# tkonolige/city2ba

Hardware: AMD Instinct MI355X
Metric: million observations/sec (project+Jacobian) (higher is better)
Workload: dtype f64

## Files before the change

city2ba_amd/csrc/capi_problem.hpp:

```cpp


struct c2b_problem {
    int device = 0;
    hipStream_t stream = nullptr;
    int64_t n_cam = 0, n_pts = 0, n_obs = 0;
    DevBuf<double> cam15, bal9, camblk, cen4, pts4, uv;
    DevBuf<uint32_t> cam_idx, pt_idx;
    DevBuf<char> ws;
    DevBuf<double> stats, scalar;
    int64_t shard_cam_base = 0, shard_n_cam_global = -1, shard_obs_base = 0;
    c2b_problem_options opt{0, 0, 0, 0, 0, 0, -1};
    int loss_kind = 0;
    double loss_scale = 1.0;
    int precond_kind = 0;
    int64_t precond_fallbacks = 0;
    DevBuf<uint16_t> cmask;
    DevBuf<uint8_t> pmask;
    std::vector<uint16_t> h_cmask;
    std::vector<uint8_t> h_pmask;
    int64_t const_n_cam = -1, const_n_pts = -1, const_params = 0, const_pts = 0;
    bool bal_valid = false;
    bool blk_valid = false;
    bool bal9_fresh = false;
    DevBuf<uint64_t> rows_ptr;
// ... 1273 lines not shown
    if (cam_lo < 0 || cam_hi < cam_lo || cam_hi > p->n_cam)
        return fail(C2B_ERR_INVALID_ARGUMENT, "problem_export_device: camera range [%lld, %lld) outside [0, %lld]", (long long)cam_lo,
                    (long long)cam_hi, (long long)p->n_cam);
    int rc = ensure_rows(p);
    if (rc) return rc;
    hipStream_t st = p->stream;
    uint64_t ends[2] = {0, 0};
    if (p->n_obs) {
        HIP_TRY(hipMemcpyAsync(&ends[0], p->rows_ptr + cam_lo, sizeof(uint64_t), hipMemcpyDeviceToHost, st));
        HIP_TRY(hipMemcpyAsync(&ends[1], p->rows_ptr + cam_hi, sizeof(uint64_t), hipMemcpyDeviceToHost, st));
        HIP_TRY(hipStreamSynchronize(st));
    }
    const int64_t o0 = (int64_t)ends[0], n = (int64_t)(ends[1] - ends[0]), nc = cam_hi - cam_lo;
    if (obs_lo) *obs_lo = o0;
    if (n_obs_slice) *n_obs_slice = n;
    if (cam15 && nc) HIP_TRY(hipMemcpyAsync(cam15, p->cam15 + 15 * cam_lo, sizeof(double) * 15 * (size_t)nc, hipMemcpyDeviceToDevice, st));
    if (pts4 && p->n_pts) HIP_TRY(hipMemcpyAsync(pts4, p->pts4, sizeof(double) * 4 * (size_t)p->n_pts, hipMemcpyDeviceToDevice, st));
    if (row_ptr) {
        if (p->n_obs) {
            hipLaunchKernelGGL(k_rows_rebase, dim3(blocks_of(nc + 1, 256)), dim3(256), 0, st, (const uint64_t *)(p->rows_ptr + cam_lo), nc + 1,
                               ends[0], row_ptr);
            LAUNCH_CHECK();
        } else {
            HIP_TRY(hipMemsetAsync(row_ptr, 0, sizeof(uint64_t) * (size_t)(nc + 1), st));
        }
    }
    if (pt_idx && n) HIP_TRY(hipMemcpyAsync(pt_idx, p->pt_idx + o0, sizeof(uint32_t) * (size_t)n, hipMemcpyDeviceToDevice, st));
    if (uv && n) HIP_TRY(hipMemcpyAsync(uv, p->uv + 2 * o0, sizeof(double) * 2 * (size_t)n, hipMemcpyDeviceToDevice, st));
    HIP_TRY(hipStreamSynchronize(st));
    return C2B_OK;
    C2B_API_END("problem_export_device")
}

static hipError_t compact_rows_on_device(c2b_problem *p, const uint64_t *d_row_old, const uint8_t *d_keep, const uint32_t *d_pt,
                                         const double *d_uv, int64_t n_cam, uint64_t *row_ptr_host, DevBuf<uint64_t> &row_new,
                                         DevBuf<uint32_t> &pt_new, DevBuf<double> &uv_new, int64_t *w) {
    DevBuf<uint64_t> d_tot;
    *w = 0;
    hipError_t e = d_tot.alloc((size_t)n_cam + 1);
    if (e == hipSuccess) e = row_new.alloc((size_t)n_cam + 1);
    if (e != hipSuccess) return e;
    const unsigned row_blocks = (unsigned)((n_cam + 3) / 4);
    if (n_cam) hipLaunchKernelGGL(k_keep_row_counts, dim3(row_blocks), dim3(256), 0, p->stream, d_row_old, d_keep, n_cam, d_tot);
    hipLaunchKernelGGL(k_dense_cam_scan, dim3(1), dim3(256), 0, p->stream, (const uint64_t *)d_tot, n_cam, row_new);
    e = hipMemcpyAsync(row_ptr_host, row_new, sizeof(uint64_t) * (size_t)(n_cam + 1), hipMemcpyDeviceToHost, p->stream);
    if (e == hipSuccess) e = hipStreamSynchronize(p->stream);
    if (e != hipSuccess) return e;
    *w = (int64_t)row_ptr_host[n_cam];
    e = pt_new.alloc((size_t)*w);
    if (e == hipSuccess) e = uv_new.alloc(2 * (size_t)*w);
    if (e == hipSuccess && n_cam) {
        hipLaunchKernelGGL(k_keep_row_scatter, dim3(row_blocks), dim3(256), 0, p->stream, d_row_old, (const uint64_t *)row_new, d_keep,
                           d_pt, reinterpret_cast<const double2 *>(d_uv), n_cam, pt_new, reinterpret_cast<double2 *>(uv_new.ptr));
        e = launch_error();
    }
    if (e == hipSuccess) e = hipStreamSynchronize(p->stream);
    return e;
}

int c2b_problem_visibility_pairs_compact(c2b_problem *p, int64_t n_pairs, const uint32_t *cam_idx, const uint32_t *pt_idx,
                                         double max_dist, uint64_t *row_ptr) {
    C2B_API_BEGIN
    NEED_UPLOADED(p, "problem_visibility_pairs_compact");
    if (n_pairs < 0 || !row_ptr || (n_pairs && (!cam_idx || !pt_idx)))
        return fail(C2B_ERR_INVALID_ARGUMENT, "problem_visibility_pairs_compact: bad arguments");
    for (int64_t i = 0; i < n_pairs; ++i) {
        if (cam_idx[i] >= (uint64_t)p->n_cam || pt_idx[i] >= (uint64_t)p->n_pts)
            return fail(C2B_ERR_INDEX_OUT_OF_RANGE, "problem_visibility_pairs_compact: pair %lld out of range", (long long)i);
        if (i && cam_idx[i] < cam_idx[i - 1])
            return fail(C2B_ERR_INVALID_ARGUMENT, "problem_visibility_pairs_compact: cam_idx must be non-decreasing (pair %lld)", (long long)i);
    }
    int rc = ensure_camblk(p);
    if (rc) return rc;
    free_dense(p);
    const int64_t n_cam = p->n_cam;
    const size_t n = (size_t)(n_pairs ? n_pairs : 1);
    DevBuf<uint32_t> d_c, d_p, d_pt_new;
    DevBuf<double> d_uv, d_uv_new;
    DevBuf<uint8_t> d_k;
    DevBuf<uint64_t> d_row, d_row_new;
    int64_t w = 0;
    hipError_t e = d_c.alloc(n);
    if (e == hipSuccess) e = d_p.alloc(n);
    if (e == hipSuccess) e = d_uv.alloc(2 * n);
    if (e == hipSuccess) e = d_k.alloc(n);
    if (e == hipSuccess) e = d_row.alloc((size_t)n_cam + 1);
    if (e == hipSuccess && n_pairs) e = hipMemcpyAsync(d_c, cam_idx, sizeof(uint32_t) * n, hipMemcpyHostToDevice, p->stream);
    if (e == hipSuccess && n_pairs) e = hipMemcpyAsync(d_p, pt_idx, sizeof(uint32_t) * n, hipMemcpyHostToDevice, p->stream);
    if (e == hipSuccess) {
        if (n_pairs) rc = c2b_visibility_pairs(p->camblk, p->pts4, d_c, d_p, n_pairs, max_dist, d_uv, d_k, p->stream);
        if (!rc) {
            hipLaunchKernelGGL(k_rows_from_sorted, dim3(blocks_for(n_pairs + 1)), dim3(kBlock), 0, p->stream, (const uint32_t *)d_c,
                               n_pairs, n_cam, d_row);
            e = launch_error();
            if (e == hipSuccess)
                e = compact_rows_on_device(p, d_row, d_k, d_p, d_uv, n_cam, row_ptr, d_row_new, d_pt_new, d_uv_new, &w);
        }
    }
    if (rc || e != hipSuccess) (void)hipStreamSynchronize(p->stream);
    if (!rc && e == hipSuccess) {
        p->dense_row = std::move(d_row_new); p->dense_pt = std::move(d_pt_new); p->dense_uv = std::move(d_uv_new); p->dense_n = w;
    }
    if (rc) return rc;
    if (e != hipSuccess) return fail(hip_code(e), "problem_visibility_pairs_compact: %s", hipGetErrorString(e));
    return C2B_OK;
    C2B_API_END("problem_visibility_pairs_compact")
}

int c2b_problem_visibility_within_distance(c2b_problem *p, double max_dist, int occlusion, double block_length, double block_inset,
                                           uint64_t *row_ptr) {
    C2B_API_BEGIN
    NEED_UPLOADED(p, "problem_visibility_within_distance");
    if (!(max_dist >= 0.0) || (occlusion && !(block_length > 0.0)))
        return fail(C2B_ERR_INVALID_ARGUMENT, "problem_visibility_within_distance: max_dist must be >= 0 (and block_length > 0 with occlusion)");
    const int64_t n_cam = p->n_cam, n_pts = p->n_pts;
    if (n_pts >= ((int64_t)1 << 32) || n_cam >= ((int64_t)1 << 31))
        return fail(C2B_ERR_INVALID_ARGUMENT, "problem_visibility_within_distance: too many cameras or points");
    int rc = ensure_camblk(p);
    if (rc) return rc;
    free_dense(p);
    hipStream_t st = p->stream;
    if (n_cam == 0 || n_pts == 0) {
        DevBuf<uint64_t> row0;
        DevBuf<uint32_t> pt0;
        DevBuf<double> uv0;
        hipError_t e0 = row0.alloc((size_t)n_cam + 1);
        if (e0 == hipSuccess) e0 = pt0.alloc(1);
        if (e0 == hipSuccess) e0 = uv0.alloc(2);
        if (e0 == hipSuccess) e0 = hipMemsetAsync(row0.ptr, 0, sizeof(uint64_t) * (size_t)(n_cam + 1), st);
        if (e0 == hipSuccess) e0 = hipStreamSynchronize(st);
        if (e0 != hipSuccess) return fail(C2B_ERR_HIP, "problem_visibility_within_distance: %s", hipGetErrorString(e0));
        if (row_ptr) std::fill(row_ptr, row_ptr + n_cam + 1, (uint64_t)0);
        p->dense_row = std::move(row0); p->dense_pt = std::move(pt0); p->dense_uv = std::move(uv0);
        p->dense_n = 0;
        return C2B_OK;
    }
    double stats[C2B_STATS_DOUBLES];
    rc = compute_stats(p);
    if (rc) return rc;
    HIP_TRY(hipMemcpyAsync(stats, p->stats, sizeof stats, hipMemcpyDeviceToHost, st));
    HIP_TRY(hipStreamSynchronize(st));
    CellGrid g;
    g.x0 = stats[6]; g.z0 = stats[8];
    const double ex = stats[9] - stats[6], ez = stats[11] - stats[8];
    double cs = (max_dist > 0.0 ? max_dist : 1.0) * (1.0 + 0x1.0p-20);
    if (!(ex >= 0.0) || !(ez >= 0.0) || !std::isfinite(ex) || !std::isfinite(ez) || !std::isfinite(cs))
        return fail(C2B_ERR_INVALID_ARGUMENT, "problem_visibility_within_distance: non-finite coordinates");
    auto cells = [&](double c) { return (std::floor(ex / c) + 1.0) * (std::floor(ez / c) + 1.0); };
    while (cells(cs) > (double)(1 << 24)) cs *= 2.0;
    g.inv_cs = 1.0 / cs;
    g.ncx = (int)std::floor(ex / cs) + 1; g.ncz = (int)std::floor(ez / cs) + 1;
    const int64_t n_cells = (int64_t)g.ncx * g.ncz;

    DevArena arena;
    DevBuf<uint32_t> cell_of, counts, cursor, sorted, tiles, total, cam_count, pos, max32;
    DevBuf<unsigned long long> sum64;
    DevBuf<uint64_t> row64;
    const int64_t big = std::max(n_cells + 1, n_cam + 1);
    auto temporaries = [&](auto &&each) {
        each(cell_of, (size_t)n_pts); each(counts, (size_t)(n_cells + 1)); each(cursor, (size_t)(n_cells + 1));
        each(sorted, (size_t)n_pts); each(tiles, (size_t)(big / kScanTile + 2)); each(total, (size_t)1);
        each(cam_count, (size_t)(n_cam + 1)); each(pos, (size_t)(n_cam + 1)); each(sum64, (size_t)1); each(max32, (size_t)1);
    };
    size_t arena_bytes = 0;
    temporaries([&](auto &b, size_t n) { arena_bytes += DevArena::room(b, n); });
    hipError_t e = arena.reserve(arena_bytes);
    if (e == hipSuccess) e = row64.alloc((size_t)n_cam + 1);
    if (e != hipSuccess) return fail(hip_code(e), "problem_visibility_within_distance: %s", hipGetErrorString(e));
    temporaries([&](auto &b, size_t n) { arena.carve(b, n); });

    HIP_TRY(hipMemsetAsync(counts.ptr, 0, 4 * (size_t)(n_cells + 1), st));
    HIP_TRY(hipMemsetAsync(cursor.ptr, 0, 4 * (size_t)(n_cells + 1), st));
    HIP_TRY(hipMemsetAsync(cam_count.ptr, 0, 4 * (size_t)(n_cam + 1), st));
    HIP_TRY(hipMemsetAsync(sum64.ptr, 0, 8, st));
    HIP_TRY(hipMemsetAsync(max32.ptr, 0, 4, st));
    if (n_pts) hipLaunchKernelGGL(k_cells_assign, dim3(blocks_of(n_pts, 256)), dim3(256), 0, st, reinterpret_cast<const double4 *>(p->pts4.ptr), n_pts,
                                  g, cell_of, counts);
    uint32_t n_sorted = 0, n_kept32 = 0;
    uint32_t *start = cursor;
    e = scan_flags(st, counts, n_cells + 1, start, tiles, total, &n_sorted);
    if (e == hipSuccess && (int64_t)n_sorted != n_pts) return fail(C2B_ERR_HIP, "problem_visibility_within_distance: cell counts do not add up");
    if (e == hipSuccess) e = hipMemsetAsync(counts.ptr, 0, 4 * (size_t)(n_cells + 1), st);
    if (e == hipSuccess && n_pts)
        hipLaunchKernelGGL(k_cells_fill, dim3(blocks_of(n_pts, 256)), dim3(256), 0, st, cell_of, n_pts,
                           (const uint32_t *)start, counts, sorted);
    const unsigned cam_blocks = blocks_of(n_cam, kCellWPB);
    if (e == hipSuccess && n_cam && n_pts) {
        hipLaunchKernelGGL((k_cells_visibility<false>), dim3(cam_blocks), dim3(kCellWPB * 64), 0, st, (const double *)p->camblk, n_cam,
                           reinterpret_cast<const double4 *>(p->pts4.ptr), g, (const uint32_t *)start, sorted,
                           max_dist, occlusion ? 1 : 0, block_length, block_inset, cam_count, (const uint64_t *)nullptr,
                           (uint32_t *)nullptr, (double2 *)nullptr);
        hipLaunchKernelGGL(k_sum_u32_u64, dim3(256), dim3(256), 0, st, cam_count, n_cam, sum64);
        hipLaunchKernelGGL(k_max_u32, dim3(256), dim3(256), 0, st, cam_count, n_cam, max32);
    }
    if (e == hipSuccess) e = scan_flags(st, cam_count, n_cam + 1, pos, tiles, total, &n_kept32);
    unsigned long long n_kept = 0;
    uint32_t longest = 0;
    if (e == hipSuccess) e = hipMemcpy(&n_kept, sum64.ptr, 8, hipMemcpyDeviceToHost);
    if (e == hipSuccess) e = hipMemcpy(&longest, max32.ptr, 4, hipMemcpyDeviceToHost);
    if (e == hipSuccess && n_kept != (unsigned long long)n_kept32)
        return fail(C2B_ERR_INVALID_ARGUMENT, "problem_visibility_within_distance: more than 2^32 observations");
    if (e == hipSuccess) {
        hipLaunchKernelGGL(k_widen_u32, dim3(blocks_for(n_cam + 1)), dim3(kBlock), 0, st, pos, n_cam + 1, row64);
        e = launch_error();
    }
    DevBuf<uint32_t> tmp_pt, out_pt;
    DevBuf<double2> tmp_uv;
    DevBuf<double> out_uv;
    const size_t w = (size_t)n_kept;
    if (e == hipSuccess) e = tmp_pt.alloc(w);
    if (e == hipSuccess) e = tmp_uv.alloc(w);
    if (e == hipSuccess) e = out_pt.alloc(w);
    if (e == hipSuccess) e = out_uv.alloc(2 * w);
    if (e == hipSuccess && w) {
        hipLaunchKernelGGL((k_cells_visibility<true>), dim3(cam_blocks), dim3(kCellWPB * 64), 0, st, (const double *)p->camblk, n_cam,
                           reinterpret_cast<const double4 *>(p->pts4.ptr), g, (const uint32_t *)start, sorted,
                           max_dist, occlusion ? 1 : 0, block_length, block_inset, (uint32_t *)nullptr, row64,
                           tmp_pt, tmp_uv);
        const uint32_t long_row = p->opt.rank_sort_max_row > 0 ? (uint32_t)p->opt.rank_sort_max_row : 2048u;
        if (longest <= long_row) {
            hipLaunchKernelGGL(k_rows_rank_sort, dim3(cam_blocks), dim3(kCellWPB * 64), 0, st, row64, n_cam, tmp_pt, tmp_uv, out_pt,
                               reinterpret_cast<double2 *>(out_uv.ptr));
            e = launch_error();
        } else {
            e = launch_error();
            std::vector<uint64_t> rp((size_t)n_cam + 1);
            std::vector<uint32_t> hp(w), hq(w);
            std::vector<double> hu(2 * w), hv(2 * w);
            if (e == hipSuccess) e = hipMemcpyAsync(rp.data(), row64.ptr, 8 * ((size_t)n_cam + 1), hipMemcpyDeviceToHost, st);
            if (e == hipSuccess) e = hipMemcpyAsync(hp.data(), tmp_pt.ptr, 4 * w, hipMemcpyDeviceToHost, st);
            if (e == hipSuccess) e = hipMemcpyAsync(hu.data(), tmp_uv.ptr, 16 * w, hipMemcpyDeviceToHost, st);
            if (e == hipSuccess) e = hipStreamSynchronize(st);
            if (e == hipSuccess) {
                const int T = (int)std::min<int64_t>(std::max(1u, std::thread::hardware_concurrency()), std::max<int64_t>(1, n_cam));
                c2b_host::run_threads(T, [&](int t) {
                        std::vector<uint32_t> order;
                        for (int64_t c = n_cam * t / T; c < n_cam * (t + 1) / T; ++c) {
                            const size_t b = (size_t)rp[(size_t)c], k = (size_t)(rp[(size_t)c + 1] - rp[(size_t)c]);
                            order.resize(k);
                            for (size_t i = 0; i < k; ++i) order[i] = (uint32_t)i;
                            std::sort(order.begin(), order.end(), [&](uint32_t x, uint32_t y) { return hp[b + x] < hp[b + y]; });
                            for (size_t i = 0; i < k; ++i) {
                                hq[b + i] = hp[b + order[i]];
                                hv[2 * (b + i)] = hu[2 * (b + order[i])];
                                hv[2 * (b + i) + 1] = hu[2 * (b + order[i]) + 1];
                            }
                        }
                    });
                e = hipMemcpyAsync(out_pt.ptr, hq.data(), 4 * w, hipMemcpyHostToDevice, st);
                if (e == hipSuccess) e = hipMemcpyAsync(out_uv.ptr, hv.data(), 16 * w, hipMemcpyHostToDevice, st);
                if (e == hipSuccess) e = hipStreamSynchronize(st);
            }
        }
    }
    if (e == hipSuccess && row_ptr)
        e = hipMemcpyAsync(row_ptr, row64.ptr, sizeof(uint64_t) * (size_t)(n_cam + 1), hipMemcpyDeviceToHost, st);
    if (e == hipSuccess) e = hipStreamSynchronize(st);
    if (e != hipSuccess) {
        (void)hipStreamSynchronize(st);
        return fail(hip_code(e), "problem_visibility_within_distance: %s", hipGetErrorString(e));
    }
    p->dense_row = std::move(row64); p->dense_pt = std::move(out_pt); p->dense_uv = std::move(out_uv);
    p->dense_n = (int64_t)n_kept;
    return C2B_OK;
    C2B_API_END("problem_visibility_within_distance")
}

int c2b_problem_generate_world_points(c2b_problem *p, const float *tri9, int64_t n_tri, int64_t num_points, double max_dist,
                                      uint64_t seed, int64_t *n_out) {
    C2B_API_BEGIN
    NEED_UPLOADED(p, "problem_generate_world_points");
    if (!tri9 || n_tri < 0 || num_points < 0 || !n_out || num_points >= ((int64_t)1 << 31))
        return fail(C2B_ERR_INVALID_ARGUMENT, "problem_generate_world_points: bad arguments");
    if (p->n_obs != 0) return fail(C2B_ERR_INVALID_ARGUMENT, "problem_generate_world_points: the problem already has observations");
    if (p->n_cam == 0)
        return fail(C2B_ERR_INVALID_ARGUMENT, "Cannot generate world points with 0 cameras. Try increasing the number of cameras generated (via --cameras).");
    if (n_tri == 0) return fail(C2B_ERR_INVALID_ARGUMENT, "the model has no triangles");
    int rc = ensure_camblk(p);
    if (rc) return rc;
    hipStream_t st = p->stream;
    const int64_t n_cam = p->n_cam;
    std::vector<double> cum((size_t)n_tri);
    {
        double acc = 0.0;
        for (int64_t t = 0; t < n_tri; ++t) {
            const float *q = tri9 + 9 * t;
            const double a[3] = {(double)q[3] - (double)q[0], (double)q[4] - (double)q[1], (double)q[5] - (double)q[2]};
            const double b[3] = {(double)q[6] - (double)q[0], (double)q[7] - (double)q[1], (double)q[8] - (double)q[2]};
            const double c[3] = {a[1] * b[2] - a[2] * b[1], a[2] * b[0] - a[0] * b[2], a[0] * b[1] - a[1] * b[0]};
            acc += std::sqrt((c[0] * c[0] + c[1] * c[1]) + c[2] * c[2]) / 2.0;
            cum[(size_t)t] = acc;
        }
    }
    DevBuf<float> d_tri;
    DevBuf<double> d_cum;
    const double4 *centres = reinterpret_cast<const double4 *>(p->cen4.ptr);
    hipError_t e = d_tri.alloc(9 * (size_t)n_tri);
    if (e == hipSuccess) e = d_cum.alloc((size_t)n_tri);
    if (e == hipSuccess) e = hipMemcpyAsync(d_tri.ptr, tri9, 36 * (size_t)n_tri, hipMemcpyHostToDevice, st);
    if (e == hipSuccess) e = hipMemcpyAsync(d_cum.ptr, cum.data(), 8 * (size_t)n_tri, hipMemcpyHostToDevice, st);
    if (e != hipSuccess) return fail(hip_code(e), "problem_generate_world_points: %s", hipGetErrorString(e));
    double stats[C2B_STATS_DOUBLES];
    rc = c2b_stats(p->camblk, p->cen4, n_cam, p->pts4, 0, p->ws, p->stats, st);
    if (rc) return rc;
    HIP_TRY(hipMemcpyAsync(stats, p->stats, sizeof stats, hipMemcpyDeviceToHost, st));
    HIP_TRY(hipStreamSynchronize(st));
    CellGrid g;
    g.x0 = stats[6]; g.z0 = stats[8];
    const double ex = stats[9] - stats[6], ez = stats[11] - stats[8];
    double cs = (max_dist > 0.0 ? max_dist : 1.0) * (1.0 + 0x1.0p-20);
    if (!(ex >= 0.0) || !(ez >= 0.0) || !std::isfinite(ex) || !std::isfinite(ez) || !std::isfinite(cs))
        return fail(C2B_ERR_INVALID_ARGUMENT, "problem_generate_world_points: non-finite coordinates");
    auto cells = [&](double c) { return (std::floor(ex / c) + 1.0) * (std::floor(ez / c) + 1.0); };
    while (cells(cs) > (double)(1 << 24)) cs *= 2.0;
    g.inv_cs = 1.0 / cs;
    g.ncx = (int)std::floor(ex / cs) + 1; g.ncz = (int)std::floor(ez / cs) + 1;
    const int64_t n_cells = (int64_t)g.ncx * g.ncz;
    const int64_t chunk = std::max<int64_t>(4096, std::min<int64_t>(num_points, (int64_t)1 << 20));
    DevBuf<uint32_t> cell_of, counts, startb, sorted, tiles, total, ok, pos;
    DevBuf<double4> cand;
    DevBuf<unsigned long long> cutoff;
    DevBuf<double> out;
    const int64_t big = std::max(n_cells + 1, chunk);
    e = cell_of.alloc((size_t)n_cam);
    if (e == hipSuccess) e = counts.alloc((size_t)(n_cells + 1));
    if (e == hipSuccess) e = startb.alloc((size_t)(n_cells + 1));
    if (e == hipSuccess) e = sorted.alloc((size_t)n_cam);
    if (e == hipSuccess) e = tiles.alloc((size_t)(big / kScanTile + 2));
    if (e == hipSuccess) e = total.alloc(1);
    if (e == hipSuccess) e = cand.alloc((size_t)chunk);
    if (e == hipSuccess) e = ok.alloc((size_t)chunk);
    if (e == hipSuccess) e = pos.alloc((size_t)chunk);
    if (e == hipSuccess) e = cutoff.alloc(1);
    if (e == hipSuccess) e = out.alloc(4 * (size_t)std::max<int64_t>(num_points, 1));
    if (e == hipSuccess) e = hipMemsetAsync(counts.ptr, 0, 4 * (size_t)(n_cells + 1), st);
    if (e != hipSuccess) return fail(hip_code(e), "problem_generate_world_points: %s", hipGetErrorString(e));
    hipLaunchKernelGGL(k_cells_assign, dim3(blocks_of(n_cam, 256)), dim3(256), 0, st, centres, n_cam, g, cell_of, counts);
    uint32_t n_sorted = 0;
    e = scan_flags(st, counts, n_cells + 1, startb, tiles, total, &n_sorted);
    if (e == hipSuccess && (int64_t)n_sorted != n_cam) return fail(C2B_ERR_HIP, "problem_generate_world_points: cell counts do not add up");
    if (e == hipSuccess) e = hipMemsetAsync(counts.ptr, 0, 4 * (size_t)(n_cells + 1), st);
    if (e == hipSuccess)
        hipLaunchKernelGGL(k_cells_fill, dim3(blocks_of(n_cam, 256)), dim3(256), 0, st, cell_of, n_cam, startb, counts, sorted);
    if (e == hipSuccess) e = launch_error();
    int64_t accepted = 0, failed = 0;
    const int64_t fail_threshold = 10 * num_points;
    for (int64_t k0 = 0; e == hipSuccess && accepted < num_points && failed < fail_threshold; k0 += chunk) {
        const unsigned long long all = (unsigned long long)chunk;
        e = hipMemcpyAsync(cutoff.ptr, &all, 8, hipMemcpyHostToDevice, st);
        if (e != hipSuccess) break;
        hipLaunchKernelGGL(k_world_candidates, dim3(blocks_of(chunk, 256)), dim3(256), 0, st, d_tri, n_tri, d_cum, seed, k0, chunk,
                           centres, g, startb, sorted, max_dist, cand, ok);
        uint32_t n_ok = 0;
        e = scan_flags(st, ok, chunk, pos, tiles, total, &n_ok);
        if (e != hipSuccess) break;
        hipLaunchKernelGGL(k_world_cutoff, dim3(blocks_of(chunk, 256)), dim3(256), 0, st, pos, chunk,
                           (uint64_t)(num_points - accepted), (uint64_t)(fail_threshold - failed), cutoff);
        hipLaunchKernelGGL(k_world_accept, dim3(blocks_of(chunk, 256)), dim3(256), 0, st, cand, ok, pos, chunk, cutoff,
                           reinterpret_cast<double4 *>(out.ptr) + accepted);
        e = launch_error();
        unsigned long long cut = 0;
        if (e == hipSuccess) e = hipMemcpyAsync(&cut, cutoff.ptr, 8, hipMemcpyDeviceToHost, st);
        if (e == hipSuccess) e = hipStreamSynchronize(st);
        if (e != hipSuccess) break;
        uint32_t took = n_ok;
        if ((int64_t)cut < chunk) {
            e = hipMemcpy(&took, pos + cut, 4, hipMemcpyDeviceToHost);
            if (e != hipSuccess) break;
        }
        accepted += (int64_t)took;
        failed += (int64_t)cut - (int64_t)took;
    }
    if (e != hipSuccess) return fail(C2B_ERR_HIP, "problem_generate_world_points: %s", hipGetErrorString(e));
    if (failed >= fail_threshold && num_points > 0)
        return fail(C2B_ERR_INVALID_ARGUMENT, "Failed to generate enough points. %lld successes, %lld failures, %lld requested points.",
// ... 348 lines not shown
```

city2ba_amd/csrc/cell_kernels.hpp:

```cpp
#pragma once
#include "camera_math.hpp"

namespace c2b {

struct CellGrid {
    double x0, z0, inv_cs;
    int ncx, ncz;
};

C2B_DEV int cell_coord(double v, double v0, double inv_cs, int n) {
    const double f = floor((v - v0) * inv_cs);
    return f < 0.0 ? 0 : (f >= (double)n ? n - 1 : (int)f);
}

__global__ __launch_bounds__(256) void k_cells_assign(const double4 *__restrict__ pts4, int64_t n, CellGrid g,
                                                     uint32_t *__restrict__ cell_of, uint32_t *__restrict__ counts) {
    const int64_t j = (int64_t)blockIdx.x * 256 + threadIdx.x;
    if (j >= n) return;
    const double4 p = pts4[j];
    const uint32_t c = (uint32_t)(cell_coord(p.x, g.x0, g.inv_cs, g.ncx) * g.ncz + cell_coord(p.z, g.z0, g.inv_cs, g.ncz));
    cell_of[j] = c;
    atomicAdd(counts + c, 1u);
}

__global__ __launch_bounds__(256) void k_cells_fill(const uint32_t *__restrict__ cell_of, int64_t n, const uint32_t *__restrict__ start,
                                                   uint32_t *__restrict__ cursor, uint32_t *__restrict__ sorted) {
    const int64_t j = (int64_t)blockIdx.x * 256 + threadIdx.x;
    if (j >= n) return;
    const uint32_t c = cell_of[j];
    sorted[start[c] + atomicAdd(cursor + c, 1u)] = (uint32_t)j;
}

C2B_DEV bool seg_unique_intersection(double p0x, double p0y, double p1x, double p1y, double q0x, double q0y, double q1x,
                                     double q1y, double &ix, double &iy) {
    const double rx = p1x - p0x, ry = p1y - p0y;
    const double sx = q1x - q0x, sy = q1y - q0y;
    const double r_cross_s = rx * sy - ry * sx;
    if (r_cross_s == 0.0) return false;
    const double qpx = q0x - p0x, qpy = q0y - p0y;
    const double t = qpx * (sy / r_cross_s) - qpy * (sx / r_cross_s);
    const double u = qpx * (ry / r_cross_s) - qpy * (rx / r_cross_s);
    if (!(0.0 <= t && t <= 1.0 && 0.0 <= u && u <= 1.0)) return false;
    ix = p0x + t * rx;
    iy = p0y + t * ry;
    return true;
}

C2B_DEV bool hits_in_block_dev(double sx, double sy, double ex, double ey, int64_t bix, int64_t biy, double L, double inset) {
    const double block_end = L - inset;
    const double ox = (double)bix * L, oy = (double)biy * L;
    const double lo_x = ox + inset, lo_y = oy + inset, hi_x = ox + block_end, hi_y = oy + block_end;
#pragma unroll
    for (int k = 0; k < 4; ++k) {
        const double ax = k == 2 ? hi_x : lo_x, ay = k == 3 ? hi_y : lo_y;
        const double bx = k == 0 ? lo_x : hi_x, by = k == 1 ? lo_y : hi_y;
        double px, py;
        if (seg_unique_intersection(sx, sy, ex, ey, ax, ay, bx, by, px, py)) {
            const double dx = ex - px;
            if (sqrt(dx * dx + (ey - py)) > 1e-8) return true;
        }
    }
    return false;
}

C2B_DEV bool hits_building_dev(double cx, double cz, double px, double pz, double L, double inset) {
    const int64_t cbx = (int64_t)trunc(cx / L), cby = (int64_t)trunc(cz / L);
    const int64_t pbx = (int64_t)trunc(px / L), pby = (int64_t)trunc(pz / L);
    const int64_t x0 = cbx < pbx ? cbx : pbx, x1 = cbx < pbx ? pbx : cbx;
    const int64_t y0 = cby < pby ? cby : pby, y1 = cby < pby ? pby : cby;
    for (int64_t bx = x0; bx <= x1; ++bx)
        for (int64_t by = y0; by <= y1; ++by)
            if (hits_in_block_dev(cx, cz, px, pz, bx, by, L, inset)) return true;
    return false;
}

constexpr int kCellWPB = 4;
template <bool FILL>
__global__ __launch_bounds__(kCellWPB * 64) void k_cells_visibility(
    const double *__restrict__ camblk, int64_t n_cam, const double4 *__restrict__ pts4, CellGrid g,
    const uint32_t *__restrict__ start, const uint32_t *__restrict__ sorted, double max_dist, int occlusion, double L,
    double inset, uint32_t *__restrict__ cam_count, const uint64_t *__restrict__ row_ptr, uint32_t *__restrict__ pt_out,
    double2 *__restrict__ uv_out) {
    const int lane = threadIdx.x & 63;
    const int64_t c = (int64_t)blockIdx.x * kCellWPB + __builtin_amdgcn_readfirstlane(threadIdx.x >> 6);
    if (c >= n_cam) return;
    const CamRec cam(camblk, c);
    const double gx = cam[kCenter], gy = cam[kCenter + 1], gz = cam[kCenter + 2];
    const int ccx = cell_coord(gx, g.x0, g.inv_cs, g.ncx), ccz = cell_coord(gz, g.z0, g.inv_cs, g.ncz);
    const double r2 = max_dist * max_dist;
    uint64_t dst = FILL ? row_ptr[c] : 0;
    uint32_t count = 0;
    const int ix0 = ccx > 0 ? ccx - 1 : 0, ix1 = ccx + 1 < g.ncx ? ccx + 1 : g.ncx - 1;
    const int iz0 = ccz > 0 ? ccz - 1 : 0, iz1 = ccz + 1 < g.ncz ? ccz + 1 : g.ncz - 1;
    for (int ix = ix0; ix <= ix1; ++ix) {
        const uint32_t b = start[ix * g.ncz + iz0], e = start[ix * g.ncz + iz1 + 1];
        for (uint32_t k0 = b; k0 < e; k0 += 64) {
            const uint32_t k = k0 + lane;
            const bool valid = k < e;
            const uint32_t j = sorted[valid ? k : e - 1];
            const double4 X = pts4[j];
            const double dx = gx - X.x, dy = gy - X.y, dz = gz - X.z;
            const double d2 = dot3(dx, dy, dz, dx, dy, dz);
            bool keep = valid && d2 <= r2;
            double u = 0.0, v = 0.0;
            if (keep) {
                const Proj p = project_obs(cam, X.x, X.y, X.z);
                u = p.u; v = p.v;
                keep = sqrt(d2) < max_dist && p.qz <= 0.0 && u >= -1.0 && u <= 1.0 && v >= -1.0 && v <= 1.0;
            }
            if (keep && occlusion) keep = !hits_building_dev(gx, gz, X.x, X.z, L, inset);
            const uint64_t m = __builtin_amdgcn_ballot_w64(keep);
            if (FILL && keep) {
                const uint64_t at = dst + (uint64_t)__builtin_popcountll(m & ((1ull << lane) - 1ull));
                pt_out[at] = j;
                uv_out[at] = make_double2(u, v);
            }
            const uint32_t got = (uint32_t)__builtin_popcountll(m);
            count += got;
            dst += got;
        }
    }
    if (!FILL && lane == 0) cam_count[c] = count;
}

__global__ __launch_bounds__(kCellWPB * 64) void k_rows_rank_sort(const uint64_t *__restrict__ row_ptr, int64_t n_cam,
                                                                const uint32_t *__restrict__ pt_in, const double2 *__restrict__ uv_in,
                                                                uint32_t *__restrict__ pt_out, double2 *__restrict__ uv_out) {
    const int lane = threadIdx.x & 63;
    const int64_t c = (int64_t)blockIdx.x * kCellWPB + __builtin_amdgcn_readfirstlane(threadIdx.x >> 6);
    if (c >= n_cam) return;
    const uint64_t b = row_ptr[c], e = row_ptr[c + 1];
    for (uint64_t i0 = b; i0 < e; i0 += 64) {
        const uint64_t i = i0 + lane;
        const bool valid = i < e;
        const uint32_t mine = pt_in[valid ? i : e - 1];
        uint32_t rank = 0;
        for (uint64_t j = b; j < e; ++j) rank += pt_in[j] < mine ? 1u : 0u;
        if (valid) {
            pt_out[b + rank] = mine;
            uv_out[b + rank] = uv_in[i];
        }
    }
}

__global__ __launch_bounds__(256) void k_max_u32(const uint32_t *__restrict__ v, int64_t n, uint32_t *__restrict__ out) {
    uint32_t m = 0;
    for (int64_t i = (int64_t)blockIdx.x * 256 + threadIdx.x; i < n; i += (int64_t)gridDim.x * 256) m = v[i] > m ? v[i] : m;
#pragma unroll
    for (int off = 32; off > 0; off >>= 1) { const uint32_t o = __shfl_down(m, off, 64); m = o > m ? o : m; }
    if ((threadIdx.x & 63) == 0 && m) atomicMax(out, m);
}

__global__ __launch_bounds__(256) void k_sum_u32_u64(const uint32_t *__restrict__ v, int64_t n, unsigned long long *__restrict__ out) {
    unsigned long long s = 0;
    for (int64_t i = (int64_t)blockIdx.x * 256 + threadIdx.x; i < n; i += (int64_t)gridDim.x * 256) s += v[i];
#pragma unroll
    for (int off = 32; off > 0; off >>= 1) s += __shfl_down(s, off, 64);
    if ((threadIdx.x & 63) == 0 && s) atomicAdd(out, s);
}

struct GridDirs { double m[4][9]; };

C2B_DEV void grid_slot(int64_t n, int64_t B, int64_t slots, int per, int64_t &bx, int64_t &by, int64_t &i, int &k, bool &along_x) {
    const int64_t row_full = slots * per * (2 * B + 1);
    if (n < B * row_full) {
        bx = n / row_full;
        const int64_t r = n % row_full;
        if (r < 2 * per * slots * B) {
            by = r / (2 * per * slots);
            const int64_t r2 = r % (2 * per * slots);
            i = r2 / (2 * per);
            const int kk = (int)(r2 % (2 * per));
            along_x = kk < per; k = kk % per;
        } else {
            by = B;
            const int64_t r2 = r - 2 * per * slots * B;
            i = r2 / per; k = (int)(r2 % per); along_x = true;
        }
    } else {
        bx = B;
        const int64_t r = n - B * row_full;
        by = r / (per * slots);
        const int64_t r2 = r % (per * slots);
        i = r2 / per; k = (int)(r2 % per); along_x = false;
    }
}

__global__ __launch_bounds__(256) void k_grid_cameras(int64_t n_cam, int64_t cpb, int64_t B, double L, double cam_h, GridDirs d,
                                                     double *__restrict__ cam15) {
    const int64_t n = (int64_t)blockIdx.x * 256 + threadIdx.x;
    if (n >= n_cam) return;
    int64_t bx, by, i;
    int k;
    bool along_x;
    grid_slot(n, B, cpb, 2, bx, by, i, k, along_x);
    const double offset_x = L * (double)bx, offset_z = L * (double)by;
    const double t = (double)i / (double)cpb * L;
    const double px = along_x ? offset_x + t : offset_x, pz = along_x ? offset_z : offset_z + t;
    const double *R = d.m[(along_x ? 0 : 2) + k];
    double v[3];
    cm_mat_vec(R, px, cam_h, pz, v);
    double *o = cam15 + 15 * n;
#pragma unroll
    for (int q = 0; q < 9; ++q) o[q] = R[q];
    o[9] = -1.0 * v[0]; o[10] = -1.0 * v[1]; o[11] = -1.0 * v[2];
    o[12] = 1.0; o[13] = 0.0; o[14] = 0.0;
}

__global__ __launch_bounds__(256) void k_grid_points(int64_t n_pts, int64_t ppb, int64_t B, double L, double inset, double pt_h,
                                                    double4 *__restrict__ pts4) {
    const int64_t n = (int64_t)blockIdx.x * 256 + threadIdx.x;
    if (n >= n_pts) return;
    int64_t bx, by, i;
    int k;
    bool along_x;
    grid_slot(n, B, ppb, 6, bx, by, i, k, along_x);
    const double offset_x = L * (double)bx, offset_z = L * (double)by;
    const double step = (L - inset * 2.0) / (double)ppb;
    const double loc = (along_x ? offset_x : offset_z) + inset + (double)i * step;
    const double a = k < 2 ? loc : loc + step / 2.0;
    const double o = along_x ? offset_z : offset_x;
    const double half = inset / 2.0;
    const double c = k == 0 || k == 2 ? o - inset : (k == 1 || k == 3 ? o + inset : (k == 4 ? o - half : o + half));
    const double y = k < 2 ? pt_h : 0.0;
    pts4[n] = along_x ? make_double4(a, y, c, 0.0) : make_double4(c, y, a, 0.0);
}

__global__ __launch_bounds__(256) void k_line_layout(int64_t n_cam, int64_t n_pts, double length, double point_offset, double cam_h,
                                                    double pt_h, GridDirs d, double *__restrict__ cam15, double4 *__restrict__ pts4) {
    const int64_t n = (int64_t)blockIdx.x * 256 + threadIdx.x;
    if (n < n_cam) {
        const double *R = d.m[2];
        double v[3];
        cm_mat_vec(R, 0.0, cam_h, (double)n * length / (double)(n_cam - 1), v);
        double *o = cam15 + 15 * n;
#pragma unroll
        for (int q = 0; q < 9; ++q) o[q] = R[q];
        o[9] = -1.0 * v[0]; o[10] = -1.0 * v[1]; o[11] = -1.0 * v[2];
        o[12] = 1.0; o[13] = 0.0; o[14] = 0.0;
    }
    if (n < n_pts) {
        const double z = (double)(n / 2) * length / (double)(n_pts / 2 - 1);
        pts4[n] = make_double4((n % 2 == 0) ? -point_offset : point_offset, pt_h, z, 0.0);
    }
}

C2B_DEV uint64_t bswap64(uint64_t v) { return __builtin_bswap64(v); }

__global__ __launch_bounds__(256) void k_bbal_rows(const uint64_t *__restrict__ row_ptr, int64_t n_cam, int64_t n_pts, int64_t n_obs,
                                                  uint64_t *__restrict__ img) {
    const int64_t c = (int64_t)blockIdx.x * 256 + threadIdx.x;
    if (c == 0) { img[0] = bswap64((uint64_t)n_cam); img[1] = bswap64((uint64_t)n_pts); img[2] = bswap64((uint64_t)n_obs); }
    if (c >= n_cam) return;
    const uint64_t b = row_ptr ? row_ptr[c] : 0, e = row_ptr ? row_ptr[c + 1] : 0;
    img[3 + c + 3 * b] = bswap64(e - b);
}
__global__ __launch_bounds__(256) void k_bbal_observations(const uint32_t *__restrict__ cam_idx, const uint32_t *__restrict__ pt_idx,
                                                          const double2 *__restrict__ uv, int64_t n_obs, uint64_t *__restrict__ img) {
    const int64_t o = (int64_t)blockIdx.x * 256 + threadIdx.x;
    if (o >= n_obs) return;
    const double2 q = uv[o];
    uint64_t *w = img + 3 + ((uint64_t)cam_idx[o] + 1) + 3 * (uint64_t)o;
    w[0] = bswap64((uint64_t)pt_idx[o]);
    w[1] = bswap64((uint64_t)__double_as_longlong(q.x));
    w[2] = bswap64((uint64_t)__double_as_longlong(q.y));
}
__global__ __launch_bounds__(256) void k_bbal_rows_f64(const double *__restrict__ in, int64_t n, int width, int stride,
                                                      uint64_t *__restrict__ out) {
    const int64_t i = (int64_t)blockIdx.x * 256 + threadIdx.x;
    if (i >= n * width) return;
    const int64_t r = i / width, k = i % width;
    out[i] = bswap64((uint64_t)__double_as_longlong(in[r * stride + k]));
}

__global__ __launch_bounds__(256) void k_bbal_read_observations(const uint64_t *__restrict__ raw, const uint32_t *__restrict__ cam_idx,
                                                               int64_t n_obs, uint64_t n_pts, uint32_t *__restrict__ pt_idx,
                                                               double2 *__restrict__ uv, uint32_t *__restrict__ bad) {
    const int64_t o = (int64_t)blockIdx.x * 256 + threadIdx.x;
    if (o >= n_obs) return;
    const uint64_t *w = raw + 3 + ((uint64_t)cam_idx[o] + 1) + 3 * (uint64_t)o;
    const uint64_t pt = bswap64(w[0]);
    if (pt >= n_pts) atomicOr(bad, 1u);
    pt_idx[o] = (uint32_t)pt;
    uv[o] = make_double2(__longlong_as_double((long long)bswap64(w[1])), __longlong_as_double((long long)bswap64(w[2])));
}
__global__ __launch_bounds__(256) void k_bbal_read_rows_f64(const uint64_t *__restrict__ in, int64_t n, int width, int stride,
                                                           double *__restrict__ out) {
    const int64_t i = (int64_t)blockIdx.x * 256 + threadIdx.x;
    if (i >= n * stride) return;
    const int64_t r = i / stride, k = i % stride;
// ... 68 lines not shown
```

Before: 27700.

## Stage short visibility rows during count pass to skip second fill pass

The counting pass of the cell visibility kernel now also writes up to `cap` kept observations per camera into a fixed-stride staging buffer. The fill pass then reruns only for cameras whose rows overflow the cap, and the rank sort reads each row from staging or the overflow buffer as appropriate. This is meant to avoid recomputing projections and occlusion tests for most cameras, at the cost of a staging buffer sized n_cam*cap, chosen from free device memory. The code touched is the visibility-building setup, which may not be part of the timed project+Jacobian metric.

```diff
diff --git a/city2ba_amd/csrc/capi_problem.hpp b/city2ba_amd/csrc/capi_problem.hpp
--- a/city2ba_amd/csrc/capi_problem.hpp
+++ b/city2ba_amd/csrc/capi_problem.hpp
@@ -1449,8 +1449,17 @@
     g.ncx = (int)std::floor(ex / cs) + 1; g.ncz = (int)std::floor(ez / cs) + 1;
     const int64_t n_cells = (int64_t)g.ncx * g.ncz;
 
+    uint32_t cap = 64;
+    {
+        size_t free_b = 0, total_b = 0;
+        HIP_TRY(hipMemGetInfo(&free_b, &total_b));
+        while (cap && (double)n_cam * (double)cap * 20.0 > (double)free_b / 4.0) cap /= 2;
+    }
+    const size_t n_stage = (size_t)n_cam * cap;
+
     DevArena arena;
-    DevBuf<uint32_t> cell_of, counts, cursor, sorted, tiles, total, cam_count, pos, max32;
+    DevBuf<uint32_t> cell_of, counts, cursor, sorted, tiles, total, cam_count, pos, max32, stage_pt;
+    DevBuf<double2> stage_uv;
     DevBuf<unsigned long long> sum64;
     DevBuf<uint64_t> row64;
     const int64_t big = std::max(n_cells + 1, n_cam + 1);
@@ -1458,6 +1467,7 @@
         each(cell_of, (size_t)n_pts); each(counts, (size_t)(n_cells + 1)); each(cursor, (size_t)(n_cells + 1));
         each(sorted, (size_t)n_pts); each(tiles, (size_t)(big / kScanTile + 2)); each(total, (size_t)1);
         each(cam_count, (size_t)(n_cam + 1)); each(pos, (size_t)(n_cam + 1)); each(sum64, (size_t)1); each(max32, (size_t)1);
+        each(stage_uv, n_stage); each(stage_pt, n_stage);
     };
     size_t arena_bytes = 0;
     temporaries([&](auto &b, size_t n) { arena_bytes += DevArena::room(b, n); });
@@ -1486,7 +1496,7 @@
         hipLaunchKernelGGL((k_cells_visibility<false>), dim3(cam_blocks), dim3(kCellWPB * 64), 0, st, (const double *)p->camblk, n_cam,
                            reinterpret_cast<const double4 *>(p->pts4.ptr), g, (const uint32_t *)start, sorted,
                            max_dist, occlusion ? 1 : 0, block_length, block_inset, cam_count, (const uint64_t *)nullptr,
-                           (uint32_t *)nullptr, (double2 *)nullptr);
+                           cap, stage_pt, stage_uv);
         hipLaunchKernelGGL(k_sum_u32_u64, dim3(256), dim3(256), 0, st, cam_count, n_cam, sum64);
         hipLaunchKernelGGL(k_max_u32, dim3(256), dim3(256), 0, st, cam_count, n_cam, max32);
     }
@@ -1501,23 +1511,27 @@
         hipLaunchKernelGGL(k_widen_u32, dim3(blocks_for(n_cam + 1)), dim3(kBlock), 0, st, pos, n_cam + 1, row64);
         e = launch_error();
     }
+    const uint32_t long_row = p->opt.rank_sort_max_row > 0 ? (uint32_t)p->opt.rank_sort_max_row : 2048u;
+    const bool host_sort = longest > long_row;
+    const uint32_t fill_above = host_sort ? 0u : cap;
     DevBuf<uint32_t> tmp_pt, out_pt;
     DevBuf<double2> tmp_uv;
     DevBuf<double> out_uv;
     const size_t w = (size_t)n_kept;
-    if (e == hipSuccess) e = tmp_pt.alloc(w);
-    if (e == hipSuccess) e = tmp_uv.alloc(w);
+    if (e == hipSuccess && longest > fill_above) e = tmp_pt.alloc(w);
+    if (e == hipSuccess && longest > fill_above) e = tmp_uv.alloc(w);
     if (e == hipSuccess) e = out_pt.alloc(w);
     if (e == hipSuccess) e = out_uv.alloc(2 * w);
     if (e == hipSuccess && w) {
-        hipLaunchKernelGGL((k_cells_visibility<true>), dim3(cam_blocks), dim3(kCellWPB * 64), 0, st, (const double *)p->camblk, n_cam,
-                           reinterpret_cast<const double4 *>(p->pts4.ptr), g, (const uint32_t *)start, sorted,
-                           max_dist, occlusion ? 1 : 0, block_length, block_inset, (uint32_t *)nullptr, row64,
-                           tmp_pt, tmp_uv);
-        const uint32_t long_row = p->opt.rank_sort_max_row > 0 ? (uint32_t)p->opt.rank_sort_max_row : 2048u;
-        if (longest <= long_row) {
-            hipLaunchKernelGGL(k_rows_rank_sort, dim3(cam_blocks), dim3(kCellWPB * 64), 0, st, row64, n_cam, tmp_pt, tmp_uv, out_pt,
-                               reinterpret_cast<double2 *>(out_uv.ptr));
+        if (longest > fill_above)
+            hipLaunchKernelGGL((k_cells_visibility<true>), dim3(cam_blocks), dim3(kCellWPB * 64), 0, st, (const double *)p->camblk, n_cam,
+                               reinterpret_cast<const double4 *>(p->pts4.ptr), g, (const uint32_t *)start, sorted,
+                               max_dist, occlusion ? 1 : 0, block_length, block_inset, cam_count, row64, fill_above,
+                               tmp_pt, tmp_uv);
+        if (!host_sort) {
+            hipLaunchKernelGGL(k_rows_rank_sort, dim3(cam_blocks), dim3(kCellWPB * 64), 0, st, row64, n_cam, cap,
+                               (const uint32_t *)stage_pt, (const double2 *)stage_uv, (const uint32_t *)tmp_pt, (const double2 *)tmp_uv,
+                               out_pt, reinterpret_cast<double2 *>(out_uv.ptr));
             e = launch_error();
         } else {
             e = launch_error();
diff --git a/city2ba_amd/csrc/cell_kernels.hpp b/city2ba_amd/csrc/cell_kernels.hpp
--- a/city2ba_amd/csrc/cell_kernels.hpp
+++ b/city2ba_amd/csrc/cell_kernels.hpp
@@ -79,16 +79,19 @@
 __global__ __launch_bounds__(kCellWPB * 64) void k_cells_visibility(
     const double *__restrict__ camblk, int64_t n_cam, const double4 *__restrict__ pts4, CellGrid g,
     const uint32_t *__restrict__ start, const uint32_t *__restrict__ sorted, double max_dist, int occlusion, double L,
-    double inset, uint32_t *__restrict__ cam_count, const uint64_t *__restrict__ row_ptr, uint32_t *__restrict__ pt_out,
-    double2 *__restrict__ uv_out) {
+    double inset, uint32_t *__restrict__ cam_count, const uint64_t *__restrict__ row_ptr, uint32_t cap,
+    uint32_t *__restrict__ pt_out, double2 *__restrict__ uv_out) {
     const int lane = threadIdx.x & 63;
     const int64_t c = (int64_t)blockIdx.x * kCellWPB + __builtin_amdgcn_readfirstlane(threadIdx.x >> 6);
     if (c >= n_cam) return;
+    if (FILL && cam_count[c] <= cap) return;
     const CamRec cam(camblk, c);
     const double gx = cam[kCenter], gy = cam[kCenter + 1], gz = cam[kCenter + 2];
     const int ccx = cell_coord(gx, g.x0, g.inv_cs, g.ncx), ccz = cell_coord(gz, g.z0, g.inv_cs, g.ncz);
     const double r2 = max_dist * max_dist;
-    uint64_t dst = FILL ? row_ptr[c] : 0;
+    const uint64_t row0 = FILL ? row_ptr[c] : (uint64_t)c * cap;
+    uint32_t *__restrict__ const pt_row = pt_out + row0;
+    double2 *__restrict__ const uv_row = uv_out + row0;
     uint32_t count = 0;
     const int ix0 = ccx > 0 ? ccx - 1 : 0, ix1 = ccx + 1 < g.ncx ? ccx + 1 : g.ncx - 1;
     const int iz0 = ccz > 0 ? ccz - 1 : 0, iz1 = ccz + 1 < g.ncz ? ccz + 1 : g.ncz - 1;
@@ -110,32 +113,35 @@
             }
             if (keep && occlusion) keep = !hits_building_dev(gx, gz, X.x, X.z, L, inset);
             const uint64_t m = __builtin_amdgcn_ballot_w64(keep);
-            if (FILL && keep) {
-                const uint64_t at = dst + (uint64_t)__builtin_popcountll(m & ((1ull << lane) - 1ull));
-                pt_out[at] = j;
-                uv_out[at] = make_double2(u, v);
+            const uint32_t at = count + (uint32_t)__builtin_popcountll(m & ((1ull << lane) - 1ull));
+            if (keep && (FILL || at < cap)) {
+                pt_row[at] = j;
+                uv_row[at] = make_double2(u, v);
             }
-            const uint32_t got = (uint32_t)__builtin_popcountll(m);
-            count += got;
-            dst += got;
+            count += (uint32_t)__builtin_popcountll(m);
         }
     }
     if (!FILL && lane == 0) cam_count[c] = count;
 }
 
-__global__ __launch_bounds__(kCellWPB * 64) void k_rows_rank_sort(const uint64_t *__restrict__ row_ptr, int64_t n_cam,
-                                                                const uint32_t *__restrict__ pt_in, const double2 *__restrict__ uv_in,
+__global__ __launch_bounds__(kCellWPB * 64) void k_rows_rank_sort(const uint64_t *__restrict__ row_ptr, int64_t n_cam, uint32_t cap,
+                                                                const uint32_t *__restrict__ stage_pt, const double2 *__restrict__ stage_uv,
+                                                                const uint32_t *__restrict__ over_pt, const double2 *__restrict__ over_uv,
                                                                 uint32_t *__restrict__ pt_out, double2 *__restrict__ uv_out) {
     const int lane = threadIdx.x & 63;
     const int64_t c = (int64_t)blockIdx.x * kCellWPB + __builtin_amdgcn_readfirstlane(threadIdx.x >> 6);
     if (c >= n_cam) return;
-    const uint64_t b = row_ptr[c], e = row_ptr[c + 1];
-    for (uint64_t i0 = b; i0 < e; i0 += 64) {
+    const uint64_t b = row_ptr[c], n = row_ptr[c + 1] - b;
+    const bool staged = n <= (uint64_t)cap;
+    const uint64_t in0 = staged ? (uint64_t)c * cap : b;
+    const uint32_t *__restrict__ pt_in = (staged ? stage_pt : over_pt) + in0;
+    const double2 *__restrict__ uv_in = (staged ? stage_uv : over_uv) + in0;
+    for (uint64_t i0 = 0; i0 < n; i0 += 64) {
         const uint64_t i = i0 + lane;
-        const bool valid = i < e;
-        const uint32_t mine = pt_in[valid ? i : e - 1];
+        const bool valid = i < n;
+        const uint32_t mine = pt_in[valid ? i : n - 1];
         uint32_t rank = 0;
-        for (uint64_t j = b; j < e; ++j) rank += pt_in[j] < mine ? 1u : 0u;
+        for (uint64_t j = 0; j < n; ++j) rank += pt_in[j] < mine ? 1u : 0u;
         if (valid) {
             pt_out[b + rank] = mine;
             uv_out[b + rank] = uv_in[i];
```

After: 27500. No clear change (-0.7%).
